# nsbuitrago/parasail-rs

Hardware: AMD Instinct MI355X
Metric: GCUPS (cell updates/s) local-affine SW, 1M 150x150 pairs, 1/2/4/8 GPUs (higher is better)
Workload: dtype int16

## Files before the change

parasail-rs_amd/csrc/pmx_sw16.hip:

```cpp
#include "pmx_common.h"
#include "pmx_switches.h"
#include "pmx_pk16.h"
#include <cstdlib>

__device__ __forceinline__ v2s pk_adds(v2s a, v2s b) { return __builtin_elementwise_add_sat(a, b); }
__device__ __forceinline__ v2s pk_subs(v2s a, v2s b) { return __builtin_elementwise_sub_sat(a, b); }
__device__ __forceinline__ v2s pk_max(v2s a, v2s b) { return __builtin_elementwise_max(a, b); }

#ifndef PMX_SHARE_PERIOD
#define PMX_SHARE_PERIOD 16
#endif
#define FLOOR2 0x80008000

template <int G, int R, int VAR>
__global__ __launch_bounds__(64, (VAR == 6 && R <= 20) ? 4 : 1)
void pmx_sw16_kernel(const uint8_t *__restrict__ qbuf, const int64_t *__restrict__ qoff,
                     const uint8_t *__restrict__ rbuf, const int64_t *__restrict__ roff,
                     long long n, const int16_t *__restrict__ gmat, const uint8_t *__restrict__ gmap,
                     int msize, int open, int ext, int RP ,
                     int q_shared ,
                     int limit ,
                     const unsigned *__restrict__ perm,
                     const int *__restrict__ n_dev ,
                     unsigned *__restrict__ retry_list, int *__restrict__ retry_count ,
                     int sat_above ,
                     uint32_t *__restrict__ tbuf, int Tmax ,
                     pmx_record_t *__restrict__ out)
{
    if (n_dev) n = *n_dev;
    if ((long long)blockIdx.x * (2 * (64 / G)) >= n) return;
    constexpr bool M3 = VAR >= 1;
    constexpr bool V2 = VAR >= 2;
    constexpr bool PT = VAR == 6;
    constexpr bool TR = VAR == 7;
    static_assert(!TR || R == 16, "trace: four packed planes of 4 rows");
    constexpr bool FETCH = VAR == 8;
    constexpr bool U8 = VAR == 3 || VAR == 5 || PT || TR || FETCH;
    constexpr bool SK = VAR >= 4;
    constexpr int EB = U8 ? 1 : 2;
    constexpr int WR = U8 ? 4 : 2;
    constexpr int RS = (R + WR - 1) / WR * WR;
    constexpr int QP = G * RS;
    constexpr int QP2 = QP / 2;
    constexpr int SLOTS = 64 / G;
    constexpr int NP = 2 * SLOTS;
    extern __shared__ __attribute__((aligned(16))) unsigned char lds[];

    const int lane = threadIdx.x;
    constexpr bool IL = G == 8 && VAR != 7;
    const int g = IL ? (lane % 16) / 2 : lane % G;
    const int slot = IL ? (lane / 16) * 2 + (lane & 1) : lane / G;
    const int PROF_STRIDE = PT ? 0 : msize * QP * EB;

    constexpr int PT_TABS = 32;
    int16_t *prof = reinterpret_cast<int16_t *>(lds);
    unsigned char *rsym = lds + (PT ? PT_TABS : NP * PROF_STRIDE + QP * EB);
    int16_t *mat = reinterpret_cast<int16_t *>(rsym + (FETCH ? 0 : NP * RP));
    unsigned char *map = reinterpret_cast<unsigned char *>(mat + msize * msize);
    long long *ptab = reinterpret_cast<long long *>(map + 256 + ((8 - ((msize * msize * 2) & 7)) & 7));

    typedef __attribute__((address_space(3))) int *lds_int;
    auto tab_at = [](int byte) -> int { return *(lds_int)(uintptr_t)byte; };
    constexpr int QS = (G * R + 3) / 4 * 4;
    unsigned char *qsym = reinterpret_cast<unsigned char *>(ptab + 5 * NP);

    const long long pair0 = (long long)blockIdx.x * NP;

    for (int i = lane; i < msize * msize; i += 64) mat[i] = gmat[i];
    for (int i = lane; i < 256; i += 64) map[i] = gmap[i];
    if (lane < NP) {
        long long pos = pair0 + lane; if (pos >= n) pos = n - 1;
        const long long pi = perm ? (long long)perm[pos] : pos;
        const long long qb = q_shared ? 0 : qoff[pi], rb = roff[pi];
        ptab[5 * lane + 0] = qb;
        ptab[5 * lane + 1] = q_shared ? q_shared : (qoff[pi + 1] - qb);
        ptab[5 * lane + 2] = rb;
        ptab[5 * lane + 3] = roff[pi + 1] - rb;
        ptab[5 * lane + 4] = (pair0 + lane < n) ? pi : -1;
    }
    __syncthreads();
    const uint8_t *qbase = qbuf;
    const uint8_t *rbase = rbuf;

    int max_rlen = 0;
#pragma unroll
    for (int p = 0; p < NP; ++p) max_rlen = max(max_rlen, (int)ptab[5 * p + 3]);
    constexpr int UB = NP < 8 ? NP : 8;
    for (int p0 = 0; p0 < (FETCH ? 0 : NP); p0 += UB) {
        for (int j0 = 0; j0 < RP; j0 += 64) {
            const int j = j0 + lane, jr = j - (G - 1);
            unsigned char raw[UB]; bool ok[UB];
#pragma unroll
            for (int u = 0; u < UB; ++u) {
                const int p = p0 + u;
                ok[u] = jr >= 0 && jr < (int)ptab[5 * p + 3];
                raw[u] = ok[u] ? rbase[ptab[5 * p + 2] + jr] : (unsigned char)0;
            }
            if (j < RP) {
#pragma unroll
                for (int u = 0; u < UB; ++u) {
                    const int p = p0 + u;
                    if (PT)
                        rsym[(p >> 1) * 2 * RP + 2 * j + (p & 1)] = (unsigned char)(4 * (ok[u] ? map[raw[u]] : msize));
                    else
                        rsym[p * RP + j] = ok[u] ? map[raw[u]] : (unsigned char)((NP - p) * msize);
                }
            }
        }
    }

    if (PT) {
        for (int p0 = 0; p0 < NP; p0 += UB) {
            for (int j0 = 0; j0 < QS; j0 += 64) {
                const int j = j0 + lane;
                unsigned char raw[UB]; bool ok[UB];
#pragma unroll
                for (int u = 0; u < UB; ++u) {
                    const int p = p0 + u;
                    ok[u] = j < (int)ptab[5 * p + 1];
                    raw[u] = ok[u] ? qbase[ptab[5 * p + 0] + j] : (unsigned char)0;
                }
                if (j < QS) {
#pragma unroll
                    for (int u = 0; u < UB; ++u) qsym[(p0 + u) * QS + j] = ok[u] ? map[raw[u]] : (unsigned char)0xFF;
                }
            }
        }
    }

    constexpr int QITEMS = PT ? 0 : (NP * QP2 + 63) / 64;
    constexpr int QB = QITEMS < 5 ? (QITEMS < 1 ? 1 : QITEMS) : 5;
    for (int it0 = 0; it0 < QITEMS; it0 += QB) {
        unsigned char r0[QB], r1[QB]; bool v0[QB], v1[QB];
#pragma unroll
        for (int u = 0; u < QB; ++u) {
            const int item = (it0 + u) * 64 + lane;
            const int p = min(item / QP2, NP - 1), rp = item - p * QP2;
            const int ql = (int)ptab[5 * p + 1];
            const uint8_t *qp = qbase + ptab[5 * p + 0];
            const int p0 = 2 * rp, p1 = 2 * rp + 1;
            const int k0 = p0 % RS, k1 = p1 % RS;
            const int row0 = (p0 / RS) * R + k0, row1 = (p1 / RS) * R + k1;
            v0[u] = item < NP * QP2 && k0 < R && row0 < ql; v1[u] = item < NP * QP2 && k1 < R && row1 < ql;
            r0[u] = v0[u] ? qp[row0] : (unsigned char)0;
            r1[u] = v1[u] ? qp[row1] : (unsigned char)0;
        }
#pragma unroll
        for (int u = 0; u < QB; ++u) {
            const int item = (it0 + u) * 64 + lane;
            if (it0 + u < QITEMS && item < NP * QP2) {
                const int p = item / QP2, rp = item - p * QP2;
                const int q0 = v0[u] ? map[r0[u]] : -1;
                const int q1 = v1[u] ? map[r1[u]] : -1;
                for (int sym = 0; sym < msize; ++sym) {
                    const int s0 = ((q0 < 0) ? 0 : mat[q0 * msize + sym]) + (V2 ? open : 0);
                    const int s1 = ((q1 < 0) ? 0 : mat[q1 * msize + sym]) + (V2 ? open : 0);
                    if (U8) {
                        reinterpret_cast<unsigned short *>(lds + p * PROF_STRIDE + sym * QP)[rp] =
                            (unsigned short)((s0 & 0xFF) | ((s1 & 0xFF) << 8));
                    } else {
                        int *pp = reinterpret_cast<int *>(prof) + p * (PROF_STRIDE / 4) + rp;
                        pp[sym * QP2] = (s0 & 0xFFFF) | (s1 << 16);
                    }
                }
            }
        }
    }
    if (!PT) {
        for (int idx = lane; idx < QP * EB / 4; idx += 64)
            reinterpret_cast<int *>(lds + NP * PROF_STRIDE)[idx] = V2 ? 0 : FLOOR2;
    }
    int sel[R];
    int wild = 0;
    if (PT) {
        if (lane <= msize) {
            int v = 0;
            if (lane < msize)
                for (int k = 0; k < 4 && k < msize; ++k) v |= ((mat[k * msize + lane] + open) & 0xFF) << (8 * k);
            ((lds_int)(uintptr_t)0)[lane] = v;
        }
    }
    __syncthreads();
    if (PT) {
        const unsigned char *qa = qsym + (2 * slot) * QS + g * R, *qb = qa + QS;
#pragma unroll
        for (int k = 0; k < R; ++k) {
            const int ca = qa[k], cb = qb[k];
            wild |= ((ca >= 4 && ca != 0xFF) ? 1 : 0) | ((cb >= 4 && cb != 0xFF) ? 2 : 0);
            sel[k] = (ca < 4 ? ca : 0x0C) | 0x0C00 | ((cb < 4 ? 4 + cb : 0x0C) << 16) | 0x0C000000;
        }
        asm volatile("" : "+v"(wild));
    }
    __syncthreads();

    const int pA = 2 * slot, pB = 2 * slot + 1;
    const unsigned char *profA = lds + pA * PROF_STRIDE + g * (RS * EB);
    const unsigned char *profB = lds + pB * PROF_STRIDE + g * (RS * EB);
    constexpr int SS = PT ? 2 : 1;
    const unsigned char *rsA = PT ? rsym + slot * 2 * RP + 2 * ((G - 1) - g) : rsym + pA * RP + (G - 1) - g;
    const unsigned char *rsB = PT ? rsA + 1 : rsym + pB * RP + (G - 1) - g;
    const int SYMSTRIDE = QP * EB;

    const v2s vOpen = PK((open & 0xFFFF) | (open << 16));
    const v2s vExt = PK((ext & 0xFFFF) | (ext << 16));
    constexpr int ZERO2 = M3 ? PK16_SW_BIAS2 : FLOOR2;
    const v2s vZero = PK(ZERO2);

    v2s HA[R], HB[R], E[R], Hsave[R];
    const int skew0 = SK ? (((G - g) * ext) & 0xFFFF) * 0x00010001 : 0;
    const v2s vC = PK(I32(vOpen) - I32(vExt));
    const v2s vInitH = V2 ? PK(ZERO2 - I32(vOpen) + skew0) : vZero;
#pragma unroll
    for (int k = 0; k < R; ++k) { HA[k] = vInitH; HB[k] = vInitH; E[k] = V2 ? vInitH : (M3 ? PK(0) : vZero); Hsave[k] = vZero; }
    v2s best = PK(ZERO2 + skew0 - (SK ? I32(vC) : 0));
    int bestcol = g * 0x00010001;
    int vprev = 0, fake = 0;
    int Zv = ZERO2 + skew0 + I32(vExt);
    const int HNEUTRAL = V2 ? ZERO2 - I32(vOpen) : ZERO2;
    int Hout = SK ? Zv - I32(vExt) - I32(vOpen) : HNEUTRAL, Fout = SK ? Zv - I32(vExt) : ZERO2;
    v2s diag0 = PK(SK ? I32(vInitH) : HNEUTRAL);

    auto load_scores = [&](int symA, int symB, int (&wa)[RS / WR], int (&wb)[RS / WR]) {
        if (PT) { wa[0] = tab_at(symA); wb[0] = tab_at(symB); return; }
        const int *sa = reinterpret_cast<const int *>(profA + symA * SYMSTRIDE);
        const int *sb = reinterpret_cast<const int *>(profB + symB * SYMSTRIDE);
#pragma unroll
        for (int k = 0; k < RS / WR; ++k) { wa[k] = sa[k]; wb[k] = sb[k]; }
    };
    const size_t t_ss = 4;
    uint32_t *tw = TR ? tbuf + ((size_t)blockIdx.x * Tmax) * 256 + (size_t)lane * Tmax * 4 : nullptr;
    auto push = [&](v2s &pl, v2s a, v2s b) {
        const v2us fifteen = {15, 15};
        const int bit = I32(__builtin_bit_cast(v2s, __builtin_bit_cast(v2us, a - b) >> fifteen));
        int r;
        asm("v_pk_mad_u16 %0, %1, %2, %3" : "=v"(r) : "v"(I32(pl)), "v"(0x00020002), "v"(bit));
        pl = PK(r);
    };
    auto step = [&](const v2s (&Hold)[R], v2s (&Hnew)[R], const int (&wa)[RS / WR], const int (&wb)[RS / WR], int t) {
        const int Hin = group_shift_up<G, IL>(Hout, SK ? Zv - I32(vOpen) : HNEUTRAL, g);
        const int Fin = group_shift_up<G, IL>(Fout, SK ? Zv : ZERO2, g);
        v2s F = PK(Fin);
        v2s colmax = SK ? PK(0) : vZero;
        v2s Hcur[R];
        v2s Tpre[R], Epre[R];
        v2s plane[TR ? R / 4 : 1];
        if (TR) {
#pragma unroll
            for (int x = 0; x < R / 4; ++x) plane[x] = PK(0);
        }
        if (V2) {
#pragma unroll
            for (int k = 0; k < R; ++k) {
                const v2s s = PT ? PK(__builtin_amdgcn_perm(wb[0], wa[0], (unsigned)sel[k]))
                            : U8 ? PK(__builtin_amdgcn_perm(wb[k / 4], wa[k / 4], 0x0C000C00u | (unsigned)(k & 3) | ((4u + (unsigned)(k & 3)) << 16)))
                               : PK(__builtin_amdgcn_perm(wb[k / 2], wa[k / 2], (k & 1) ? 0x07060302 : 0x05040100));
                const v2s d = (k == 0) ? diag0 : Hold[k - 1];
                Tpre[k] = PK(I32(d) + I32(s));
                if (!SK) Epre[k] = PK(I32(E[k]) - I32(vExt));
            }
            __builtin_amdgcn_sched_barrier(0);
        }
#pragma unroll
        for (int k = 0; k < R; ++k) {
            const v2s s = PT ? PK(__builtin_amdgcn_perm(wb[0], wa[0], (unsigned)sel[k]))
                        : U8 ? PK(__builtin_amdgcn_perm(wb[k / 4], wa[k / 4], 0x0C000C00u | (unsigned)(k & 3) | ((4u + (unsigned)(k & 3)) << 16)))
                               : PK(__builtin_amdgcn_perm(wb[k / 2], wa[k / 2], (k & 1) ? 0x07060302 : 0x05040100));
            const v2s d = (k == 0) ? diag0 : Hold[k - 1];
            v2s H;
            if (SK) {
                const v2s Fe = PK(I32(F) - I32(vExt));
                H = pk_max3(Tpre[k], E[k], Fe);
                const v2s X = PK(I32(H) - I32(vC));
                if (TR) {
                    push(plane[k / 4], Tpre[k], H);
                    push(plane[k / 4], Fe, H);
                    push(plane[k / 4], E[k], X);
                    push(plane[k / 4], Fe, X);
                }
                E[k] = pk_max3(E[k], X, X);
                F = pk_max3(Fe, X, PK(Zv));
                Hnew[k] = X;
                if (k & 1) colmax = pk_max3(colmax, Hnew[k - 1], X);
                else if (k == R - 1) colmax = pk_max3(colmax, X, best);
            } else if (V2) {
                H = pk_max3(Tpre[k], E[k], F);
                const v2s Ho = PK(I32(H) - I32(vOpen));
                E[k] = pk_max3(Epre[k], Ho, Ho);
                F = pk_max3(PK(I32(F) - I32(vExt)), Ho, vZero);
                Hnew[k] = Ho;
                Hcur[k] = H;
                if (k & 1) colmax = pk_max3(colmax, Hcur[k - 1], H);
                else if (k == R - 1) colmax = pk_max3(colmax, H, H);
            } else if (M3) {
                const v2s Tt = PK(I32(__builtin_bit_cast(v2us, d) + __builtin_bit_cast(v2us, s)));
                H = pk_max3(Tt, E[k], F);
                const v2s Ho = pk_subus(H, vOpen);
                E[k] = pk_max3(pk_subus(E[k], vExt), Ho, Ho);
                F = pk_max3(pk_subus(F, vExt), Ho, vZero);
                Hnew[k] = H;
                if (k & 1) colmax = pk_max3(colmax, Hnew[k - 1], H);
                else if (k == R - 1) colmax = pk_max3(colmax, H, H);
            } else {
                H = pk_adds(d, s);
                H = pk_max(H, E[k]);
                H = pk_max(H, F);
                const v2s Ho = pk_subs(H, vOpen);
                E[k] = pk_max(pk_subs(E[k], vExt), Ho);
                F = pk_max(pk_subs(F, vExt), Ho);
                Hnew[k] = H;
                colmax = pk_max(colmax, H);
            }
        }
        if (TR) {
            uint4 w;
            w.x = __builtin_amdgcn_perm(I32(plane[0]), I32(plane[1]), 0x00010405);
            w.y = __builtin_amdgcn_perm(I32(plane[2]), I32(plane[3]), 0x00010405);
            w.z = __builtin_amdgcn_perm(I32(plane[0]), I32(plane[1]), 0x02030607);
            w.w = __builtin_amdgcn_perm(I32(plane[2]), I32(plane[3]), 0x02030607);
            *reinterpret_cast<uint4 *>(tw + (size_t)t * t_ss) = w;
        }
        diag0 = PK(Hin);
        Hout = I32(Hnew[R - 1]);
        Fout = I32(F);
        constexpr bool FOLDED = SK && (R & 1);
        const v2s nb = FOLDED ? colmax : M3 ? pk_max3(best, colmax, colmax) : pk_max(best, colmax);
        auto improved = [&]() -> int {
            const v2s dd = FOLDED ? (best - nb) : M3 ? (best - colmax) : pk_subs(best, colmax);
            const v2s sh = {15, 15};
            return I32(dd >> sh);
        };
        int m = FOLDED ? 0 : improved();
        if (__builtin_amdgcn_ballot_w64(FOLDED ? I32(nb) != I32(best) : m != 0) != 0) {
            if (FOLDED) m = improved();
            asm("v_bfi_b32 %0, %1, %2, %3" : "=v"(bestcol) : "v"(m), "s"((t & 0xFFFF) * 0x00010001), "v"(bestcol));
            fake &= ~m;
#pragma unroll
            for (int k = 0; k < R; ++k) Hsave[k] = PK(bfi(m, I32((V2 && !SK) ? Hcur[k] : Hnew[k]), I32(Hsave[k])));
        }
        best = SK ? PK(I32(nb) + I32(vExt)) : nb;
        if (SK) Zv += I32(vExt);
    };

    const int T = __builtin_amdgcn_readfirstlane(max_rlen) + G - 1;
    int w0a[RS / WR], w0b[RS / WR], w1a[RS / WR], w1b[RS / WR];
    const int rlA_ = (int)ptab[5 * pA + 3], rlB_ = (int)ptab[5 * pB + 3];
    const uint8_t *refA = rbase + ptab[5 * pA + 2], *refB = rbase + ptab[5 * pB + 2];
    auto fetch = [&](int x, int &ra, int &rb) {
        const int col = x - g;
        ra = (col >= 0 && col < rlA_) ? (int)refA[col] : -1;
        rb = (col >= 0 && col < rlB_) ? (int)refB[col] : -1;
    };
    auto symA_of = [&](int raw) -> int { return raw < 0 ? (NP - pA) * msize : (int)map[raw]; };
    auto symB_of = [&](int raw) -> int { return raw < 0 ? (NP - pB) * msize : (int)map[raw]; };
    int m2a = 0, m2b = 0, m3a = 0, m3b = 0, nsA, nsB;
    if (FETCH) {
        int r0a, r0b, r1a, r1b;
        fetch(0, r0a, r0b); fetch(1, r1a, r1b); fetch(2, m2a, m2b); fetch(3, m3a, m3b);
        load_scores(symA_of(r0a), symB_of(r0b), w0a, w0b);
        nsA = symA_of(r1a); nsB = symB_of(r1b);
    } else {
        load_scores(rsA[0], rsB[0], w0a, w0b);
        nsA = rsA[SS]; nsB = rsB[SS];
    }
    constexpr int SHP = PMX_SHARE_PERIOD > G ? PMX_SHARE_PERIOD : G;
    auto share_bound = [&]() {
        const int v = group_max3<G, IL>(I32(best) - skew0);
        const int fresh = v - 0x00010001 + skew0;
        const int old = vprev ? vprev + ((SHP * ext) & 0xFFFF) * 0x00010001 + skew0 : 0;
        const v2s nbest = pk_max3(best, PK(fresh), PK(old));
        fake |= pk_lt(best, nbest);
        best = nbest;
        vprev = v;
    };
    const unsigned char *rcur = rsA;
    for (int t = 0; t + 1 < T; t += 2) {
        if (SK && G > 1 && (t & (SHP - 1)) == 0 && t) share_bound();
        load_scores(nsA, nsB, w1a, w1b);
        if (FETCH) { nsA = symA_of(m2a); nsB = symB_of(m2b); fetch(t + 4, m2a, m2b); }
        else if (PT) { nsA = rcur[2 * SS]; nsB = rcur[2 * SS + 1]; asm("" : "+v"(nsA), "+v"(nsB)); }
        else { nsA = rsA[t + 2]; nsB = rsB[t + 2]; }
        __builtin_amdgcn_sched_barrier(0);
        step(HA, HB, w0a, w0b, t);
        __builtin_amdgcn_sched_barrier(0);
        load_scores(nsA, nsB, w0a, w0b);
        if (FETCH) { nsA = symA_of(m3a); nsB = symB_of(m3b); fetch(t + 5, m3a, m3b); }
        else if (PT) { nsA = rcur[3 * SS]; nsB = rcur[3 * SS + 1]; asm("" : "+v"(nsA), "+v"(nsB)); rcur += 2 * SS; }
        else { nsA = rsA[t + 3]; nsB = rsB[t + 3]; }
        __builtin_amdgcn_sched_barrier(0);
        step(HB, HA, w1a, w1b, t + 1);
        __builtin_amdgcn_sched_barrier(0);
    }
    if (T & 1) step(HA, HB, w0a, w0b, T - 1);

    unsigned long long keyA, keyB;
    {
        const int bA = (short)(I32(best) & 0xFFFF), bB = (short)(I32(best) >> 16);
        const unsigned stA = bestcol & 0xFFFF, stB = (unsigned)bestcol >> 16;
        const unsigned cA = stA - g, cB = stB - g;
        const int tA = SK ? bA - (T - (int)stA) * ext : bA, tB = SK ? bB - (T - (int)stB) * ext : bB;
        int kA = 0, kB = 0;
#pragma unroll
        for (int k = R - 1; k >= 0; --k) {
            if ((short)(I32(Hsave[k]) & 0xFFFF) == tA) kA = k;
            if ((short)(I32(Hsave[k]) >> 16) == tB) kB = k;
        }
        const int unskew = SK ? (G - g + T) * ext - (open - ext) : 0;
        const unsigned sA = (unsigned)(bA - unskew - (M3 ? PK16_SW_BIAS : -32768)), sB = (unsigned)(bB - unskew - (M3 ? PK16_SW_BIAS : -32768));
        const unsigned rA = g * R + kA, rB = g * R + kB;
        keyA = ((unsigned long long)sA << 32) | ((0xFFFFu - cA) << 16) | (0xFFFFu - rA);
        keyB = ((unsigned long long)sB << 32) | ((0xFFFFu - cB) << 16) | (0xFFFFu - rB);
        if (fake & 0xFFFF) keyA = 0;
        if (fake >> 16) keyB = 0;
    }
#pragma unroll
    for (int off = G / 2; off >= 1; off >>= 1) {
        const int lo = IL ? 2 * off : off;
        const unsigned long long oa = __shfl_xor(keyA, lo, 64), ob = __shfl_xor(keyB, lo, 64);
        keyA = oa > keyA ? oa : keyA;
        keyB = ob > keyB ? ob : keyB;
        if (PT) wild |= __shfl_xor(wild, lo, 64);
    }
    if (g == 0) {
#pragma unroll
        for (int h = 0; h < 2; ++h) {
            const long long pi = ptab[5 * (2 * slot + h) + 4];
            if (pi >= 0) {
                const unsigned long long key = h ? keyB : keyA;
                pmx_record_t rec;
                rec.score = (int)(key >> 32);
                rec.end_ref = 0xFFFF - (int)((key >> 16) & 0xFFFF);
                rec.end_query = 0xFFFF - (int)(key & 0xFFFF);
                if (M3) rec.flags = (rec.score + PK16_SW_BIAS >= limit) ? PMX_FLAG_RERUN : 0;
                else rec.flags = rec.score > 32767 ? PMX_FLAG_SATURATED : 0;
                if (rec.score > sat_above) rec.flags |= PMX_FLAG_SATURATED;
                if (PT && ((wild >> h) & 1)) {
                    rec.flags = PMX_FLAG_RETRY16;
                    retry_list[atomicAdd(retry_count, 1)] = (unsigned)pi;
                }
                out[pi] = rec;
            }
        }
    }
}


template <int G, int R, int VAR>
static int launch_one(const PmxBatch &b, const PmxDevMatrix &m, int open, int ext,
                      pmx_record_t *d_out, hipStream_t stream, const int *n_dev = nullptr, uint32_t *tbuf = nullptr, int Tmax = 0)
{
    constexpr bool PT = VAR == 6;
    constexpr int EB = (VAR == 3 || VAR == 5 || VAR == 7 || VAR == 8 || PT) ? 1 : 2, WR = 4 / EB, RS = (R + WR - 1) / WR * WR;
    constexpr int QP = G * RS, NP = 2 * (64 / G);
    if (NP * m.msize > 255) return 1;
    const int RP = ((b.max_rlen + 2 * (G - 1) + 4 + 7) / 4) * 4;
    const size_t lds = (PT ? (size_t)NP * ((G * R + 3) / 4 * 4) : (size_t)NP * m.msize * QP * EB + (size_t)QP * EB) + (VAR == 8 ? 0 : (size_t)NP * RP) +
                       (size_t)m.msize * m.msize * 2 + 256 + 8 + (size_t)NP * 40 + 32;
    if (lds > 160 * 1024) return 1;
    { const int rc = pmx_ensure_lds_attr(reinterpret_cast<const void *>(&pmx_sw16_kernel<G, R, VAR>)); if (rc) return rc; }
    const long long blocks = (b.n + NP - 1) / NP;
    if (blocks <= 0) return 0;
    if (PT) {
        hipError_t e = hipMemsetAsync(b.retry_count, 0, sizeof(int), stream);
        if (e != hipSuccess) return -(int)e;
    }
    hipLaunchKernelGGL((pmx_sw16_kernel<G, R, VAR>), dim3((unsigned)blocks), dim3(64), lds, stream,
                       b.qbuf, b.qoff, b.rbuf, b.roff, (long long)b.n, m.scores, m.mapper,
                       m.msize, open, ext, RP, b.q_shared, PK16_RERUN_LIMIT(m.max) - (VAR >= 4 ? (b.max_rlen + 2 * G + 4) * ext : 0), b.perm,
                       n_dev, b.retry_list, b.retry_count, b.sat_above > 0 ? b.sat_above : 2147483647, tbuf, Tmax, d_out);
    hipError_t e = hipGetLastError();
    if (e != hipSuccess) return -(int)e;
    if (PT) {
        PmxBatch r = b;
        r.perm = b.retry_list;
        return launch_one<G, R, 5>(r, m, open, ext, d_out, stream, b.retry_count);
    }
    return 0;
}

static bool sw16_trace_ok(const PmxBatch &b, const PmxDevMatrix &m, int open, int ext)
{
    if (pmx_env("PMX_TRACE16_GEN1") || pmx_env("PMX_SW16_NO_SKEW") || pmx_env("PMX_SW16_NO_U8") || pmx_env("PMX_SW16_VARIANT")) return false;
    if (m.msize > PMX_MAX_FAST_MSIZE || open < ext || ext < 0 || open > 1024 || b.max_rlen > 30000 || b.q_shared || b.perm) return false;
    if (m.min < -1024 || m.max > 2048 || m.min + open < 0 || open + ext > 1024 || m.max + open > 255) return false;
    const long long feasible = (long long)(b.max_qlen < b.max_rlen ? b.max_qlen : b.max_rlen) * (m.max > 0 ? m.max : 0);
    return feasible + PK16_SW_BIAS < (long long)PK16_RERUN_LIMIT(m.max) - (long long)(b.max_rlen + 2 * 64 + 4) * ext;
}
int pmx_sw16_trace_plan(const PmxBatch &b, const PmxDevMatrix &m, int open, int ext, int *variant, int *Tmax, size_t *trace_bytes)
{
    if (m.pssm) return 1;
    if (!sw16_trace_ok(b, m, open, ext)) return 1;
    if (m.msize > 8 && m.msize < 32 && !pmx_env("PMX_SW16_NO_MATRIX_LOOKUP")) {
        int G = 0;
        for (int v = 1; v < 4 && !G; ++v) if (b.max_qlen <= (8 << v) * 16) { *variant = 4 + v; G = 8 << v; }
        if (!G) return 1;
        *Tmax = (b.max_rlen + G - 1 + 1 + 15) & ~15;
        *trace_bytes = (size_t)((b.n + 2 * (64 / G) - 1) / (2 * (64 / G))) * (size_t)*Tmax * 64 * 16;
        return 0;
    }
    int G = 0;
    for (int v = 0; v < 4 && !G; ++v) {
        const int g = 8 << v, np = 2 * (64 / g);
        const size_t lds = (size_t)np * m.msize * g * 16 + (size_t)g * 16 + (size_t)np * (b.max_rlen + 2 * g + 12) +
                           (size_t)m.msize * m.msize * 2 + 256 + 8 + (size_t)np * 40 + 32;
        if (b.max_qlen <= g * 16 && np * m.msize <= 255 && lds <= 160 * 1024) { *variant = v; G = g; }
    }
    if (!G) return 1;
    const int NP = 2 * (64 / G);
    *Tmax = (b.max_rlen + G - 1 + 15) & ~15;
    *trace_bytes = (size_t)((b.n + NP - 1) / NP) * (size_t)*Tmax * 64 * 16;
    return 0;
}
int pmx_launch_sw16_trace(int variant, const PmxBatch &b, const PmxDevMatrix &m, int open, int ext,
                          pmx_record_t *d_out, uint32_t *tbuf, int Tmax, hipStream_t stream)
{
    if (m.pssm) return 1;
    if (!sw16_trace_ok(b, m, open, ext)) return 1;
    if (variant >= 4) return pmx_launch_sw16m_trace(variant - 4, b, m, open, ext, d_out, tbuf, Tmax, stream);
    switch (variant) {
    case 0: return launch_one<8, 16, 7>(b, m, open, ext, d_out, stream, nullptr, tbuf, Tmax);
    case 1: return launch_one<16, 16, 7>(b, m, open, ext, d_out, stream, nullptr, tbuf, Tmax);
    case 2: return launch_one<32, 16, 7>(b, m, open, ext, d_out, stream, nullptr, tbuf, Tmax);
    case 3: return launch_one<64, 16, 7>(b, m, open, ext, d_out, stream, nullptr, tbuf, Tmax);
    }
    return 1;
}

int pmx_launch_sw16(const PmxBatch &b, const PmxDevMatrix &m, int open, int ext,
                    pmx_record_t *d_out, hipStream_t stream, const char **kernel_name)
{
    if (m.msize > PMX_MAX_FAST_MSIZE) return 1;
    if (open < 0 || ext < 0 || open > 32767 || ext > 32767) return 1;
    if (m.max > 32767 || m.min < -32767) return 1;
    if (b.max_rlen > 60000) return 1;
    const int q = b.max_qlen;
    const char *force = pmx_env("PMX_SW16_VARIANT");
    int var = 0;
    if (open <= 1024 && ext <= 1024 && m.min >= -1024 && m.max <= 2048) var = 1;
    if (var == 1 && m.min + open >= 0 && open + ext <= 1024) var = 2;
    if (force && atoi(force) < var) var = atoi(force);
    const bool u8ok = var == 2 && m.max + open <= 255 && !pmx_env("PMX_SW16_NO_U8");
    const long long feasible = (long long)(b.max_qlen < b.max_rlen ? b.max_qlen : b.max_rlen) * (m.max > 0 ? m.max : 0);
    const bool sk = var == 2 && open >= ext && !pmx_env("PMX_SW16_NO_SKEW") &&
                    feasible + PK16_SW_BIAS < (long long)PK16_RERUN_LIMIT(m.max) - (long long)(b.max_rlen + 2 * 64 + 4) * ext;
    if (m.pssm) return (b.q_shared && var == 2 && u8ok && sk) ? pmx_launch_sw16q(b, m, open, ext, d_out, stream, kernel_name) : 1;
    const bool pt = sk && u8ok && m.msize <= 5 && b.retry_list && b.retry_count && !b.q_has_wildcard && !pmx_env("PMX_SW16_NO_PERMTABLE");
    if (b.q_shared && var == 2 && u8ok && sk && !pt) {
        const int rc = pmx_launch_sw16q(b, m, open, ext, d_out, stream, kernel_name);
        if (rc <= 0) return rc;
    }
    if (!b.q_shared && var == 2 && u8ok && sk && !pt && (m.msize > 8 || pmx_env("PMX_SW16_MATRIX_LOOKUP")) && b.n > 2048) {
        const int rc = pmx_launch_sw16m(b, m, open, ext, d_out, stream, kernel_name);
        if (rc <= 0) return rc;
    }
    const bool longref = b.max_rlen >= 1024 && !pmx_env("PMX_SW16_NO_FETCH");
#define TRY(GG, RR, NAME)                                                       \
    if (q <= (GG) * (RR)) {                                                     \
        constexpr int R4 = (RR);             \
        const bool u8 = u8ok;                                                   \
        int rc = pt ? launch_one<GG, RR, 6>(b, m, open, ext, d_out, stream)     \
               : (u8 && sk && longref) ? launch_one<GG, R4, 8>(b, m, open, ext, d_out, stream)  \
               : (u8 && sk) ? launch_one<GG, R4, 5>(b, m, open, ext, d_out, stream)  \
               : u8 ? launch_one<GG, R4, 3>(b, m, open, ext, d_out, stream)     \
               : (var == 2 && sk) ? launch_one<GG, RR, 4>(b, m, open, ext, d_out, stream)  \
               : var == 2 ? launch_one<GG, RR, 2>(b, m, open, ext, d_out, stream)  \
               : var == 1 ? launch_one<GG, RR, 1>(b, m, open, ext, d_out, stream)  \
                          : launch_one<GG, RR, 0>(b, m, open, ext, d_out, stream); \
        if (rc <= 0) { if (kernel_name) *kernel_name = pt ? NAME "/max3+vop2+skew+permtable" : var == 2 ? (sk ? ((u8 && longref) ? NAME "/max3+vop2+u8+skew+fetch" : NAME "/max3+vop2+skew") : NAME "/max3+vop2") : var == 1 ? NAME "/max3" : NAME; return rc; } \
    }
#define TRY8(RR)                                                                \
    if (u8ok && q <= 8 * (RR)) {                                                \
        int rc = pt ? launch_one<8, RR, 6>(b, m, open, ext, d_out, stream)      \
               : sk ? launch_one<8, RR, 5>(b, m, open, ext, d_out, stream) : launch_one<8, RR, 3>(b, m, open, ext, d_out, stream); \
        if (rc <= 0) { if (kernel_name) *kernel_name = pt ? "pmx_sw16_kernel<8," #RR ">/max3+vop2+skew+permtable" : sk ? "pmx_sw16_kernel<8," #RR ">/max3+vop2+u8+skew" : "pmx_sw16_kernel<8," #RR ">/max3+vop2+u8"; return rc; } \
    }
    if (b.n > 2048) { TRY8(7) TRY8(10) TRY8(13) TRY8(16) TRY8(19) TRY8(20) }
#undef TRY8
#define TRYLAT(RR)                                                              \
    if (u8ok && sk && !longref && b.n <= 64 && q <= 64 * (RR)) {                \
        const int rc = launch_one<64, RR, 5>(b, m, open, ext, d_out, stream);   \
        if (rc <= 0) { if (kernel_name) *kernel_name = "pmx_sw16_kernel<64," #RR ">/max3+vop2+u8+skew"; return rc; } \
    }
    TRYLAT(2) TRYLAT(3) TRYLAT(4) TRYLAT(8)
#undef TRYLAT
    TRY(16, 10, "pmx_sw16_kernel<16,10>")
    TRY(16, 16, "pmx_sw16_kernel<16,16>")
    TRY(32, 10, "pmx_sw16_kernel<32,10>")
    TRY(32, 16, "pmx_sw16_kernel<32,16>")
    TRY(64, 16, "pmx_sw16_kernel<64,16>")
    TRY(64, 32, "pmx_sw16_kernel<64,32>")
#undef TRY
    return 1;
}
```

Baseline: 8216.

## Precompute packed query selectors in LDS and use uniform skew across group lanes

The query symbols for the PT variant are now staged directly as byte-permute selectors laid out per slot and group. Each lane reads them as uint2 words and builds sel[] with v_perm instead of per-element compares. Wildcard detection moves to a block-wide LDS bitmask set by atomicOr, which removes the shuffle reduction of the wild flags. The skew offset no longer depends on the lane's group index, so the diagonal, shift-up boundary values and unskew terms are adjusted and the share_bound max skips its per-lane skew subtraction. These changes alter score arithmetic and carry some correctness risk.

After: 8282 (median of 6 runs). No clear change (+0.8%).

```diff
diff --git a/parasail-rs_amd/csrc/pmx_sw16.hip b/parasail-rs_amd/csrc/pmx_sw16.hip
--- a/parasail-rs_amd/csrc/pmx_sw16.hip
+++ b/parasail-rs_amd/csrc/pmx_sw16.hip
@@ -61,8 +61,9 @@
 
     typedef __attribute__((address_space(3))) int *lds_int;
     auto tab_at = [](int byte) -> int { return *(lds_int)(uintptr_t)byte; };
-    constexpr int QS = (G * R + 3) / 4 * 4;
-    unsigned char *qsym = reinterpret_cast<unsigned char *>(ptab + 5 * NP);
+    constexpr int RSEL = (R + 3) / 4 * 4;
+    unsigned char *qsel = reinterpret_cast<unsigned char *>(ptab + 5 * NP);
+    unsigned *wword = reinterpret_cast<unsigned *>(qsel + SLOTS * G * RSEL * 2);
 
     const long long pair0 = (long long)blockIdx.x * NP;
 
@@ -78,6 +79,7 @@
         ptab[5 * lane + 3] = roff[pi + 1] - rb;
         ptab[5 * lane + 4] = (pair0 + lane < n) ? pi : -1;
     }
+    if (PT && lane == 0) *wword = 0;
     __syncthreads();
     const uint8_t *qbase = qbuf;
     const uint8_t *rbase = rbuf;
@@ -110,8 +112,9 @@
     }
 
     if (PT) {
+        unsigned wl = 0;
         for (int p0 = 0; p0 < NP; p0 += UB) {
-            for (int j0 = 0; j0 < QS; j0 += 64) {
+            for (int j0 = 0; j0 < G * R; j0 += 64) {
                 const int j = j0 + lane;
                 unsigned char raw[UB]; bool ok[UB];
 #pragma unroll
@@ -120,12 +123,24 @@
                     ok[u] = j < (int)ptab[5 * p + 1];
                     raw[u] = ok[u] ? qbase[ptab[5 * p + 0] + j] : (unsigned char)0;
                 }
-                if (j < QS) {
-#pragma unroll
-                    for (int u = 0; u < UB; ++u) qsym[(p0 + u) * QS + j] = ok[u] ? map[raw[u]] : (unsigned char)0xFF;
+                int c[UB];
+#pragma unroll
+                for (int u = 0; u < UB; ++u) {
+                    c[u] = map[raw[u]];
+                    if (ok[u] && c[u] >= 4) wl |= 1u << (p0 + u);
+                }
+                if (j < G * R) {
+                    const int jg = j / R;
+                    unsigned char *dst = qsel + (jg * RSEL + (j - jg * R)) * 2;
+#pragma unroll
+                    for (int u = 0; u < UB; ++u) {
+                        const int p = p0 + u;
+                        dst[(p >> 1) * (G * RSEL * 2) + (p & 1)] = (unsigned char)((ok[u] && c[u] < 4) ? 4 * (p & 1) + c[u] : 0x0C);
+                    }
                 }
             }
         }
+        if (wl) atomicOr(wword, wl);
     }
 
     constexpr int QITEMS = PT ? 0 : (NP * QP2 + 63) / 64;
@@ -171,7 +186,6 @@
             reinterpret_cast<int *>(lds + NP * PROF_STRIDE)[idx] = V2 ? 0 : FLOOR2;
     }
     int sel[R];
-    int wild = 0;
     if (PT) {
         if (lane <= msize) {
             int v = 0;
@@ -182,14 +196,15 @@
     }
     __syncthreads();
     if (PT) {
-        const unsigned char *qa = qsym + (2 * slot) * QS + g * R, *qb = qa + QS;
-#pragma unroll
-        for (int k = 0; k < R; ++k) {
-            const int ca = qa[k], cb = qb[k];
-            wild |= ((ca >= 4 && ca != 0xFF) ? 1 : 0) | ((cb >= 4 && cb != 0xFF) ? 2 : 0);
-            sel[k] = (ca < 4 ? ca : 0x0C) | 0x0C00 | ((cb < 4 ? 4 + cb : 0x0C) << 16) | 0x0C000000;
-        }
-        asm volatile("" : "+v"(wild));
+        const uint2 *qs = reinterpret_cast<const uint2 *>(qsel + (slot * G + g) * (RSEL * 2));
+        const unsigned c0C = __builtin_amdgcn_readfirstlane(0x0C0C0C0Cu);
+#pragma unroll
+        for (int k4 = 0; k4 < RSEL / 4; ++k4) {
+            const uint2 w = qs[k4];
+#pragma unroll
+            for (int x = 0; x < 4 && 4 * k4 + x < R; ++x)
+                sel[4 * k4 + x] = (int)__builtin_amdgcn_perm(c0C, x < 2 ? w.x : w.y, (x & 1) ? 0x04030402u : 0x04010400u);
+        }
     }
     __syncthreads();
 
@@ -207,7 +222,7 @@
     const v2s vZero = PK(ZERO2);
 
     v2s HA[R], HB[R], E[R], Hsave[R];
-    const int skew0 = SK ? (((G - g) * ext) & 0xFFFF) * 0x00010001 : 0;
+    const int skew0 = SK ? ((G * ext) & 0xFFFF) * 0x00010001 : 0;
     const v2s vC = PK(I32(vOpen) - I32(vExt));
     const v2s vInitH = V2 ? PK(ZERO2 - I32(vOpen) + skew0) : vZero;
 #pragma unroll
@@ -218,7 +233,7 @@
     int Zv = ZERO2 + skew0 + I32(vExt);
     const int HNEUTRAL = V2 ? ZERO2 - I32(vOpen) : ZERO2;
     int Hout = SK ? Zv - I32(vExt) - I32(vOpen) : HNEUTRAL, Fout = SK ? Zv - I32(vExt) : ZERO2;
-    v2s diag0 = PK(SK ? I32(vInitH) : HNEUTRAL);
+    v2s diag0 = PK(SK ? I32(vInitH) - I32(vExt) : HNEUTRAL);
 
     auto load_scores = [&](int symA, int symB, int (&wa)[RS / WR], int (&wb)[RS / WR]) {
         if (PT) { wa[0] = tab_at(symA); wb[0] = tab_at(symB); return; }
@@ -237,8 +252,8 @@
         pl = PK(r);
     };
     auto step = [&](const v2s (&Hold)[R], v2s (&Hnew)[R], const int (&wa)[RS / WR], const int (&wb)[RS / WR], int t) {
-        const int Hin = group_shift_up<G, IL>(Hout, SK ? Zv - I32(vOpen) : HNEUTRAL, g);
-        const int Fin = group_shift_up<G, IL>(Fout, SK ? Zv : ZERO2, g);
+        const int Hin = group_shift_up<G, IL>(Hout, SK ? Zv - I32(vExt) - I32(vOpen) : HNEUTRAL, g);
+        const int Fin = group_shift_up<G, IL>(Fout, SK ? Zv - I32(vExt) : ZERO2, g);
         v2s F = PK(Fin);
         v2s colmax = SK ? PK(0) : vZero;
         v2s Hcur[R];
@@ -255,7 +270,7 @@
                             : U8 ? PK(__builtin_amdgcn_perm(wb[k / 4], wa[k / 4], 0x0C000C00u | (unsigned)(k & 3) | ((4u + (unsigned)(k & 3)) << 16)))
                                : PK(__builtin_amdgcn_perm(wb[k / 2], wa[k / 2], (k & 1) ? 0x07060302 : 0x05040100));
                 const v2s d = (k == 0) ? diag0 : Hold[k - 1];
-                Tpre[k] = PK(I32(d) + I32(s));
+                Tpre[k] = PK(I32(d) + I32(s) + ((SK && k == 0) ? I32(vExt) : 0));
                 if (!SK) Epre[k] = PK(I32(E[k]) - I32(vExt));
             }
             __builtin_amdgcn_sched_barrier(0);
@@ -268,7 +283,7 @@
             const v2s d = (k == 0) ? diag0 : Hold[k - 1];
             v2s H;
             if (SK) {
-                const v2s Fe = PK(I32(F) - I32(vExt));
+                const v2s Fe = k == 0 ? F : PK(I32(F) - I32(vExt));
                 H = pk_max3(Tpre[k], E[k], Fe);
                 const v2s X = PK(I32(H) - I32(vC));
                 if (TR) {
@@ -364,9 +379,9 @@
     }
     constexpr int SHP = PMX_SHARE_PERIOD > G ? PMX_SHARE_PERIOD : G;
     auto share_bound = [&]() {
-        const int v = group_max3<G, IL>(I32(best) - skew0);
-        const int fresh = v - 0x00010001 + skew0;
-        const int old = vprev ? vprev + ((SHP * ext) & 0xFFFF) * 0x00010001 + skew0 : 0;
+        const int v = group_max3<G, IL>(I32(best));
+        const int fresh = v - 0x00010001;
+        const int old = vprev ? vprev + ((SHP * ext) & 0xFFFF) * 0x00010001 : 0;
         const v2s nbest = pk_max3(best, PK(fresh), PK(old));
         fake |= pk_lt(best, nbest);
         best = nbest;
@@ -404,7 +419,7 @@
             if ((short)(I32(Hsave[k]) & 0xFFFF) == tA) kA = k;
             if ((short)(I32(Hsave[k]) >> 16) == tB) kB = k;
         }
-        const int unskew = SK ? (G - g + T) * ext - (open - ext) : 0;
+        const int unskew = SK ? (G + T) * ext - (open - ext) : 0;
         const unsigned sA = (unsigned)(bA - unskew - (M3 ? PK16_SW_BIAS : -32768)), sB = (unsigned)(bB - unskew - (M3 ? PK16_SW_BIAS : -32768));
         const unsigned rA = g * R + kA, rB = g * R + kB;
         keyA = ((unsigned long long)sA << 32) | ((0xFFFFu - cA) << 16) | (0xFFFFu - rA);
@@ -418,7 +433,6 @@
         const unsigned long long oa = __shfl_xor(keyA, lo, 64), ob = __shfl_xor(keyB, lo, 64);
         keyA = oa > keyA ? oa : keyA;
         keyB = ob > keyB ? ob : keyB;
-        if (PT) wild |= __shfl_xor(wild, lo, 64);
     }
     if (g == 0) {
 #pragma unroll
@@ -433,7 +447,7 @@
                 if (M3) rec.flags = (rec.score + PK16_SW_BIAS >= limit) ? PMX_FLAG_RERUN : 0;
                 else rec.flags = rec.score > 32767 ? PMX_FLAG_SATURATED : 0;
                 if (rec.score > sat_above) rec.flags |= PMX_FLAG_SATURATED;
-                if (PT && ((wild >> h) & 1)) {
+                if (PT && ((*wword >> (2 * slot + h)) & 1)) {
                     rec.flags = PMX_FLAG_RETRY16;
                     retry_list[atomicAdd(retry_count, 1)] = (unsigned)pi;
                 }
@@ -453,7 +467,7 @@
     constexpr int QP = G * RS, NP = 2 * (64 / G);
     if (NP * m.msize > 255) return 1;
     const int RP = ((b.max_rlen + 2 * (G - 1) + 4 + 7) / 4) * 4;
-    const size_t lds = (PT ? (size_t)NP * ((G * R + 3) / 4 * 4) : (size_t)NP * m.msize * QP * EB + (size_t)QP * EB) + (VAR == 8 ? 0 : (size_t)NP * RP) +
+    const size_t lds = (PT ? (size_t)64 * ((R + 3) / 4 * 4) * 2 + 4 : (size_t)NP * m.msize * QP * EB + (size_t)QP * EB) + (VAR == 8 ? 0 : (size_t)NP * RP) +
                        (size_t)m.msize * m.msize * 2 + 256 + 8 + (size_t)NP * 40 + 32;
     if (lds > 160 * 1024) return 1;
     { const int rc = pmx_ensure_lds_attr(reinterpret_cast<const void *>(&pmx_sw16_kernel<G, R, VAR>)); if (rc) return rc; }
```
